# JohannesBuchner/massivedatans

Measured on AMD Instinct MI355X. Metric: likelihood evals/sec across N datasets per constrained draw, higher is better.
Workload: dtype f64

## Files before the change

### massivedatans_amd/csrc/mdns_geom.h

```cpp
#pragma once
#include "mdns_internal.h"

#ifdef __HIPCC__
#pragma clang fp contract(off)

namespace mdns {

static constexpr int kMaxRegDim = 8;
#define MDNS_DIM_SWITCH(ndim, LAUNCH) \
	switch ((ndim) <= kMaxRegDim ? (ndim) : 0) { \
	case 1: LAUNCH(1); break; case 2: LAUNCH(2); break; case 3: LAUNCH(3); break; \
	case 4: LAUNCH(4); break; case 5: LAUNCH(5); break; case 6: LAUNCH(6); break; \
	case 7: LAUNCH(7); break; case 8: LAUNCH(8); break; default: LAUNCH(0); break; }
#define MDNS_DIM5_SWITCH(ndim, LAUNCH) \
	switch (ndim) { case 1: LAUNCH(1); break; case 2: LAUNCH(2); break; case 3: LAUNCH(3); break; \
	                case 4: LAUNCH(4); break; default: LAUNCH(5); break; }

__device__ __forceinline__ double sq_distance(const double *a, const double *b, int ndim)
{
	double acc = 0.0;
	for (int k = 0; k < ndim; k++) {
		const double diff = a[k] - b[k];
		acc = acc + diff * diff;
	}
	return acc;
}

template <int D>
__device__ __forceinline__ double sq_distance_fixed(const double *a, const double (&c)[D])
{
	double acc = 0.0;
#pragma unroll
	for (int k = 0; k < D; k++) {
		const double diff = a[k] - c[k];
		acc = acc + diff * diff;
	}
	return acc;
}

__device__ __forceinline__ double wave_max(double v)
{
#pragma unroll
	for (int off = 32; off > 0; off >>= 1) v = fmax(v, __shfl_xor(v, off, 64));
	return v;
}
__device__ __forceinline__ double wave_min(double v)
{
#pragma unroll
	for (int off = 32; off > 0; off >>= 1) v = fmin(v, __shfl_xor(v, off, 64));
	return v;
}

__device__ __forceinline__ double min_or_skip(double a, double b)
{
	double r;
	asm("v_min_f64 %0, %1, %2" : "=v"(r) : "v"(a), "v"(b));
	return r;
}

__device__ __forceinline__ void atomic_max_nonneg(double *addr, double v)
{
	atomicMax(reinterpret_cast<unsigned long long *>(addr), (unsigned long long) __double_as_longlong(v));
}

template <int RT>
__device__ __forceinline__ void offer_rounds(double (&nearest)[RT], double d, unsigned m)
{
	const double PINF = __longlong_as_double(0x7ff0000000000000LL), NINF = __longlong_as_double((long long) 0xfff0000000000000ULL);
#pragma unroll
	for (int b = 0; b < RT; b++) {
		const double S = (m >> b & 1u) ? NINF : PINF;
		double t;
		asm("v_max_f64 %0, %1, %2" : "=v"(t) : "v"(d), "s"(S));
		nearest[b] = min_or_skip(nearest[b], t);
	}
}

template <int RT, bool AGENT_LOADS>
__device__ __forceinline__ void merge_chunks(const double *__restrict__ part, int K, int ny, int first_point,
                                             const unsigned *__restrict__ mask, int nb, double *__restrict__ round_sq,
                                             double (&wmax)[4][RT])
{
	const int lane = threadIdx.x & 63, wv = threadIdx.x >> 6;
	const int i = first_point + (threadIdx.x >> 2), yq = threadIdx.x & 3;
	double v[RT];
#pragma unroll
	for (int b = 0; b < RT; b++) v[b] = 0.0;
	const bool counts = i < K && i >= 1;
	if (counts) {
#pragma unroll
		for (int b = 0; b < RT; b++) v[b] = 1e300;
		for (int y = yq; y < ny; y += 4) {
			const double *row = part + ((size_t) y * K + i) * RT;
#pragma unroll
			for (int b = 0; b < RT; b++)
				v[b] = fmin(v[b], AGENT_LOADS ? __hip_atomic_load(row + b, __ATOMIC_RELAXED, __HIP_MEMORY_SCOPE_AGENT) : row[b]);
		}
	}
#pragma unroll
	for (int b = 0; b < RT; b++) {
		v[b] = fmin(v[b], __shfl_xor(v[b], 1, 64));
		v[b] = fmin(v[b], __shfl_xor(v[b], 2, 64));
	}
	if (counts) {
		const unsigned m = mask[i];
#pragma unroll
		for (int b = 0; b < RT; b++) if (b >= nb || (m >> b & 1u)) v[b] = 0.0;
	}
#pragma unroll
	for (int b = 0; b < RT; b++) {
		const double w = wave_max(v[b]);
		if (lane == 0) wmax[wv][b] = w;
	}
	__syncthreads();
	if (threadIdx.x < RT && threadIdx.x < nb) {
		const double w = fmax(fmax(wmax[0][threadIdx.x], wmax[1][threadIdx.x]), fmax(wmax[2][threadIdx.x], wmax[3][threadIdx.x]));
		if (w > 0.0) atomic_max_nonneg(round_sq + threadIdx.x, w);
	}
}

__device__ __forceinline__ void radius_and_threshold(double max_sq, double &radius, double &thresh)
{
	const double r = sqrt(max_sq);
	double T;
	if (!(r > 0.0)) T = 0.0;
	else if (r == __longlong_as_double(0x7ff0000000000000LL)) T = r;
	else {
		const double t0 = r * r;
		unsigned long long u = (unsigned long long) __double_as_longlong(t0);
		bool settled = false;
		if (t0 > 1e-300 && t0 < 1e300) {
			int guard = 0;
			while (sqrt(__longlong_as_double((long long) u)) < r && guard < 8) { u++; guard++; }
			while (guard < 16 && sqrt(__longlong_as_double((long long) (u - 1))) >= r) { u--; guard++; }
			settled = guard < 16 && sqrt(__longlong_as_double((long long) u)) >= r &&
			          sqrt(__longlong_as_double((long long) (u - 1))) < r;
		}
		if (!settled) {
			unsigned long long lo = 0, hi = 0x7ff0000000000000ULL;
			while (hi - lo > 1) {
				const unsigned long long mid = lo + (hi - lo) / 2;
				if (sqrt(__longlong_as_double((long long) mid)) >= r) hi = mid; else lo = mid;
			}
			u = hi;
		}
		T = __longlong_as_double((long long) u);
	}
	radius = r;
	thresh = T;
}

__device__ __forceinline__ void finish_radius(const BootstrapFinish &fin, double *rounds, int nrounds)
{
	if (!fin.counter) return;
	handover_release();
	__syncthreads();
	if (threadIdx.x >= 64) return;
	const int lane = threadIdx.x;
	unsigned ticket = 0;
	if (lane == 0) ticket = atomicAdd(fin.counter, 1u);
	if (__shfl(ticket, 0, 64) != gridDim.x - 1) return;
	handover_acquire();
	double best = 0.0;
	for (int b = lane; b < nrounds; b += 64)
		best = fmax(best, __hip_atomic_load(rounds + b, __ATOMIC_RELAXED, __HIP_MEMORY_SCOPE_AGENT));
	best = wave_max(best);
	for (int b = lane; b < nrounds; b += 64) rounds[b] = 0.0;
	if (lane != 0) return;
	double radius, thresh;
	radius_and_threshold(best, radius, thresh);
	fin.d_res->radius = radius;
	fin.d_res->thresh = thresh;
	*fin.counter = 0;
	mail_store(&fin.h_res->radius, radius);
	mail_store(&fin.h_res->thresh, thresh);
	mail_raise(&fin.h_res->seq, fin.seq);
}

template <int PTS>
__device__ __forceinline__ int slice_total(int hits, int *part)
{
	const int lane = threadIdx.x & 63, wv = threadIdx.x >> 6, pt = lane % PTS;
#pragma unroll
	for (int off = PTS; off < 64; off <<= 1) hits += __shfl_xor(hits, off, 64);
	if (lane < PTS) part[wv * PTS + pt] = hits;
	__syncthreads();
	return (part[pt] + part[PTS + pt]) + (part[2 * PTS + pt] + part[3 * PTS + pt]);
}

__device__ __forceinline__ void count_mail_raise(const CountMail &mail, unsigned nworkgroups)
{
	if (!mail.seq_at) return;
	if (threadIdx.x < 64) handover_release();
	__syncthreads();
	if (threadIdx.x != 0) return;
	const int done = atomicAdd(mail.ticket, 1);
	if (done != (int) nworkgroups - 1) return;
	__hip_atomic_store(mail.ticket, 0, __ATOMIC_RELAXED, __HIP_MEMORY_SCOPE_AGENT);
	mail_raise(mail.seq_at, mail.seq);
}

}
#endif
```

### massivedatans_amd/csrc/mdns_neighbors.hip

```cpp
#include "mdns_geom.h"
#include <cstdlib>
#include <cstring>

#pragma clang fp contract(off)

namespace mdns {

static constexpr int kBlock = 256;
static constexpr int kMaxTile = 512;
static constexpr int kRounds = 16;
static constexpr size_t kLdsBudget = 60 * 1024;

template <int SL> struct Geo {
	static constexpr int PTS = 64 / SL;
	static constexpr int NSLICE = 4 * SL;
};

template <typename T>
__device__ __forceinline__ void stage_to_lds(T *__restrict__ dst, const T *__restrict__ src, int count)
{
	constexpr int U = 8;
	for (int base = 0; base < count; base += U * kBlock) {
		T r[U];
#pragma unroll
		for (int u = 0; u < U; u++) {
			const int e = base + u * kBlock + (int) threadIdx.x;
			r[u] = src[e < count ? e : count - 1];
		}
#pragma unroll
		for (int u = 0; u < U; u++) {
			const int e = base + u * kBlock + (int) threadIdx.x;
			if (e < count) dst[e] = r[u];
		}
	}
}


template <int D, int SL>
__global__ __launch_bounds__(kBlock) void k_count_within(
    const double *__restrict__ members, int K, int ndim, double thresh_value,
    const RegionResult *__restrict__ res, const double *__restrict__ cands, int M,
    int *__restrict__ counts, int kchunk, int tile_n, int accumulate, CountMail mail)
{
	constexpr int PTS = Geo<SL>::PTS, NSLICE = Geo<SL>::NSLICE;
	const double thresh_sq = res ? res->thresh : thresh_value;
	extern __shared__ double smem[];
	double *tile = smem;
	int *part = reinterpret_cast<int *>(smem + (size_t) tile_n * ndim);
	const int lane = threadIdx.x & 63;
	const int wv = threadIdx.x >> 6;
	const int pt = lane % PTS;
	const int slice = wv * SL + lane / PTS;
	const int j = blockIdx.x * PTS + pt;
	const int jj = j < M ? j : M - 1;
	const int kbeg = blockIdx.y * kchunk;
	const int kend = min(K, kbeg + kchunk);

	double c[D > 0 ? D : 1];
	if (D > 0) {
#pragma unroll
		for (int k = 0; k < D; k++) c[k] = cands[(size_t) jj * D + k];
	}
	int hits = 0;
	for (int t0 = kbeg; t0 < kend; t0 += tile_n) {
		const int n = min(tile_n, kend - t0);
		__syncthreads();
		stage_to_lds(tile, members + (size_t) t0 * ndim, n * ndim);
		__syncthreads();
		if (D > 0) {
#pragma unroll 4
			for (int i = slice; i < n; i += NSLICE)
				hits += sq_distance_fixed<(D > 0 ? D : 1)>(tile + i * D, c) < thresh_sq ? 1 : 0;
		} else {
			const double *cj = cands + (size_t) jj * ndim;
			for (int i = slice; i < n; i += NSLICE)
				hits += sq_distance(tile + i * ndim, cj, ndim) < thresh_sq ? 1 : 0;
		}
	}
	const int total = slice_total<PTS>(hits, part);
	if (wv == 0 && lane < PTS && j < M) {
		if (accumulate) { if (total) atomicAdd(counts + j, total); }
		else if (mail.seq_at) __hip_atomic_store(counts + j, total, __ATOMIC_RELAXED, __HIP_MEMORY_SCOPE_SYSTEM);
		else counts[j] = total;
	}
	count_mail_raise(mail, gridDim.x * gridDim.y);
}

__global__ void k_pack_chosen(const double *__restrict__ chosen, int K, int nboot, int b0, int nb,
                              unsigned *__restrict__ mask, double *__restrict__ round_sq)
{
	const int i = blockIdx.x * blockDim.x + threadIdx.x;
	if (i < nb) round_sq[b0 + i] = 0.0;
	if (i >= K) return;
	const double *row = chosen + (size_t) i * nboot + b0;
	unsigned m = 0;
#pragma unroll
	for (int b = 0; b < kRounds; b++)
		if (b < nb) m |= (row[b] != 0.0 ? 1u : 0u) << b;
	mask[i] = m;
}

template <int D, bool NN, int SL, int RT>
__global__ __launch_bounds__(kBlock) void k_nearest_chosen(
    const double *__restrict__ members, int K, int ndim, const unsigned *__restrict__ mask,
    int nb, double *__restrict__ round_sq, int tile_n, BootstrapFinish fin, double *round_all, int nround_all,
    const double *__restrict__ chosen, int nboot, int b0)
{
	constexpr int PTS = Geo<SL>::PTS, NSLICE = Geo<SL>::NSLICE;
	constexpr int NR = NN ? 1 : RT;
	extern __shared__ double smem[];
	double *tile = smem;
	double *part = smem + (size_t) tile_n * ndim;
	unsigned *tmask = reinterpret_cast<unsigned *>(part + 4 * NR * PTS);

	const int lane = threadIdx.x & 63;
	const int wv = threadIdx.x >> 6;
	const int pt = lane % PTS;
	const int slice = wv * SL + lane / PTS;
	const int i = blockIdx.x * PTS + pt;
	const int ii = i < K ? i : K - 1;
	double c[D > 0 ? D : 1];
	if (D > 0) {
#pragma unroll
		for (int k = 0; k < D; k++) c[k] = members[(size_t) ii * D + k];
	}
	unsigned mymask = (NN || chosen) ? 0u : mask[ii];
	if (!NN && chosen) {
		const double *row = chosen + (size_t) ii * nboot + b0;
		double flag[NR];
#pragma unroll
		for (int b = 0; b < NR; b++) flag[b] = row[b < nb ? b : 0];
#pragma unroll
		for (int b = 0; b < NR; b++) mymask |= (b < nb && flag[b] != 0.0 ? 1u : 0u) << b;
	}

	double nearest[NR];
#pragma unroll
	for (int b = 0; b < NR; b++) nearest[b] = 1e300;

	for (int t0 = 0; t0 < K; t0 += tile_n) {
		const int n = min(tile_n, K - t0);
		__syncthreads();
		stage_to_lds(tile, members + (size_t) t0 * ndim, n * ndim);
		if (!NN && !chosen) stage_to_lds(tmask, mask + t0, n);
		if (!NN && chosen) {
			constexpr int TRIPS = kMaxTile / kBlock;
			double flag[TRIPS][NR];
#pragma unroll
			for (int t = 0; t < TRIPS; t++) {
				const int e = min((int) threadIdx.x + t * kBlock, n - 1);
				const double *row = chosen + (size_t) (t0 + e) * nboot + b0;
#pragma unroll
				for (int b = 0; b < NR; b++) flag[t][b] = row[b < nb ? b : 0];
			}
#pragma unroll
			for (int t = 0; t < TRIPS; t++) {
				const int e = (int) threadIdx.x + t * kBlock;
				unsigned m = 0;
#pragma unroll
				for (int b = 0; b < NR; b++) m |= (b < nb && flag[t][b] != 0.0 ? 1u : 0u) << b;
				if (e < n) tmask[e] = m;
			}
		}
		__syncthreads();
		auto offer = [&](int jn) {
			double d;
			if (D > 0) d = sq_distance_fixed<(D > 0 ? D : 1)>(tile + jn * D, c);
			else d = sq_distance(members + (size_t) ii * ndim, tile + jn * ndim, ndim);
			if (NN) {
				if (t0 + jn != ii) nearest[0] = fmin(nearest[0], d);
			} else {
				const int notchosen = (int) ~tmask[jn];
				const unsigned lo = (unsigned) __double2loint(d);
				const unsigned hi = (unsigned) __double2hiint(d);
#pragma unroll
				for (int b = 0; b < NR; b++) {
					const unsigned kill = (unsigned) __builtin_amdgcn_sbfe(notchosen, b, 1);
					const double cand = __hiloint2double((int) (hi | (kill & 0x7ff80000u)), (int) lo);
					nearest[b] = min_or_skip(nearest[b], cand);
				}
			}
		};
		int jn = slice;
		for (; jn + NSLICE < n; jn += 2 * NSLICE) {
			offer(jn);
			offer(jn + NSLICE);
		}
		if (jn < n) offer(jn);
	}
#pragma unroll
	for (int b = 0; b < NR; b++) {
		double v = nearest[b];
#pragma unroll
		for (int off = PTS; off < 64; off <<= 1) v = fmin(v, __shfl_xor(v, off, 64));
		if (lane < PTS) part[(wv * NR + b) * PTS + pt] = v;
	}
	__syncthreads();
	for (int b = wv; b < (NN ? 1 : nb); b += 4) {
		double v = 0.0;
		if (lane < PTS) {
			v = fmin(fmin(part[(0 * NR + b) * PTS + pt], part[(1 * NR + b) * PTS + pt]),
			         fmin(part[(2 * NR + b) * PTS + pt], part[(3 * NR + b) * PTS + pt]));
			const bool contributes = i < K && (NN ? true : (i >= 1 && !((mymask >> b) & 1u)));
			if (!contributes) v = 0.0;
		}
		v = wave_max(v);
		if (lane == 0 && v > 0.0) atomic_max_nonneg(round_sq + b, v);
	}
	finish_radius(fin, round_all, nround_all);
}

template <int D, int RT>
__global__ __launch_bounds__(kBlock) void k_nearest_uniform(
    const double *__restrict__ members, int K, const unsigned *__restrict__ mask, int kchunk, int tile_n,
    double *__restrict__ part, unsigned *__restrict__ block_tickets, int nb, double *__restrict__ round_sq,
    BootstrapFinish fin, int nround_all)
{
	extern __shared__ double smem[];
	double *tile = smem;
	double *meet = smem + (size_t) tile_n * D;
	unsigned *tmask = reinterpret_cast<unsigned *>(meet + 4 * RT * 64);
	const int lane = threadIdx.x & 63;
	const int wv = __builtin_amdgcn_readfirstlane(threadIdx.x >> 6);
	const int i = blockIdx.x * 64 + lane;
	const int ii = i < K ? i : K - 1;
	double c[D];
#pragma unroll
	for (int k = 0; k < D; k++) c[k] = members[(size_t) ii * D + k];
	double nearest[RT];
#pragma unroll
	for (int b = 0; b < RT; b++) nearest[b] = 1e300;
	const int kbeg = blockIdx.y * kchunk, kend = min(K, kbeg + kchunk);
	for (int t0 = kbeg; t0 < kend; t0 += tile_n) {
		const int n = min(tile_n, kend - t0);
		__syncthreads();
		stage_to_lds(tile, members + (size_t) t0 * D, n * D);
		stage_to_lds(tmask, mask + t0, n);
		__syncthreads();
		auto offer = [&](int jn) {
			const double d = sq_distance_fixed<D>(tile + jn * D, c);
			offer_rounds<RT>(nearest, d, (unsigned) __builtin_amdgcn_readfirstlane((int) tmask[jn]));
		};
		int jn = wv;
		for (; jn + 4 < n; jn += 8) { offer(jn); offer(jn + 4); }
		if (jn < n) offer(jn);
	}
#pragma unroll
	for (int b = 0; b < RT; b++) meet[(wv * RT + b) * 64 + lane] = nearest[b];
	__syncthreads();
	for (int e = threadIdx.x; e < RT * 64; e += kBlock) {
		const int b = e / 64, l = e % 64;
		const double v = fmin(fmin(meet[(0 * RT + b) * 64 + l], meet[(1 * RT + b) * 64 + l]),
		                      fmin(meet[(2 * RT + b) * 64 + l], meet[(3 * RT + b) * 64 + l]));
		const int p = blockIdx.x * 64 + l;
		if (p < K) { if (block_tickets) __hip_atomic_store(&part[((size_t) blockIdx.y * K + p) * RT + b], v, __ATOMIC_RELAXED, __HIP_MEMORY_SCOPE_AGENT); else part[((size_t) blockIdx.y * K + p) * RT + b] = v; }
	}
	if (!block_tickets) return;
	__shared__ int s_last;
	__shared__ double wmax[4][RT];
	handover_release();
	__syncthreads();
	if (threadIdx.x == 0) {
		const unsigned t = atomicAdd(block_tickets + blockIdx.x, 1u);
		s_last = t == gridDim.y - 1 ? 1 : 0;
		if (s_last) block_tickets[blockIdx.x] = 0;
	}
	__syncthreads();
	if (!s_last) return;
	handover_acquire();
	merge_chunks<RT, true>(part, K, (int) gridDim.y, blockIdx.x * 64, mask, nb, round_sq, wmax);
	finish_radius(fin, round_sq, nround_all);
}

template <int RT>
__global__ __launch_bounds__(kBlock) void k_nearest_finish(
    const double *__restrict__ part, int K, int ny, const unsigned *__restrict__ mask, int nb,
    double *__restrict__ round_sq, BootstrapFinish fin, int nround_all)
{
	__shared__ double wmax[4][RT];
	merge_chunks<RT, false>(part, K, ny, blockIdx.x * (kBlock / 4), mask, nb, round_sq, wmax);
	finish_radius(fin, round_sq, nround_all);
}

static int pick_tile(int ndim, size_t per_member_extra, size_t fixed_bytes)
{
	const size_t per = (size_t) ndim * sizeof(double) + per_member_extra;
	if (fixed_bytes + 16 * per > kLdsBudget) return 0;
	size_t n = (kLdsBudget - fixed_bytes) / per;
	if (n > (size_t) kMaxTile) n = kMaxTile;
	return (int) (n & ~(size_t) 15);
}

bool launch_count_within(const double *d_members, int K, int ndim, double thresh_sq,
                         const RegionResult *d_res, const double *d_cands, int M, int *d_counts, const CountMail *mail)
{
	Context *c = ctx();
	const CountMail none = {nullptr, nullptr, 0};
	const CountMail post = mail ? *mail : none;
	const size_t fixed = 4 * 64 * sizeof(int);
	const int tile_n = pick_tile(ndim, 0, fixed);
	if (tile_n <= 0) { set_error("ndim=%d too large for the member tile", ndim); return false; }
	const bool small = (M + 63) / 64 < 2 * c->num_cus;
	const bool fine = mail != nullptr && small;
	const int pts = fine ? 4 : (small ? 16 : 64);
	const int gx = (M + pts - 1) / pts;
	int want = (2 * c->num_cus + gx - 1) / gx;
	int max_split = (K + tile_n - 1) / tile_n;
	int gy = want < max_split ? want : max_split;
	if (mail) gy = 1;
	if (gy < 1) gy = 1;
	if (gy > 65535) gy = 65535;
	int kchunk = (K + gy - 1) / gy;
	kchunk = ((kchunk + tile_n - 1) / tile_n) * tile_n;
	gy = (K + kchunk - 1) / kchunk;
	const int accumulate = gy > 1 ? 1 : 0;
	if (accumulate && !MDNS_HIP(hipMemsetAsync(d_counts, 0, (size_t) M * sizeof(int), c->stream))) return false;
	const size_t lds = (size_t) tile_n * ndim * sizeof(double) + fixed;
	dim3 grid(gx, gy);
	ProfileScope prof(2);
#define COUNT_LAUNCH(D) do { if (fine) hipLaunchKernelGGL((k_count_within<D, 16>), grid, dim3(kBlock), lds, c->stream, \
		d_members, K, ndim, thresh_sq, d_res, d_cands, M, d_counts, kchunk, tile_n, accumulate, post); \
	else if (small) hipLaunchKernelGGL((k_count_within<D, 4>), grid, dim3(kBlock), lds, c->stream, \
		d_members, K, ndim, thresh_sq, d_res, d_cands, M, d_counts, kchunk, tile_n, accumulate, post); \
	else hipLaunchKernelGGL((k_count_within<D, 1>), grid, dim3(kBlock), lds, c->stream, \
		d_members, K, ndim, thresh_sq, d_res, d_cands, M, d_counts, kchunk, tile_n, accumulate, post); } while (0)
	MDNS_DIM_SWITCH(ndim, COUNT_LAUNCH)
#undef COUNT_LAUNCH
	return launched("k_count_within");
}

template <bool NN>
static bool launch_nearest(const double *d_members, int K, int ndim, const double *d_chosen,
                           int nboot, double *d_round_sq, const BootstrapFinish *finish,
                           const unsigned *d_packed = nullptr)
{
	Context *c = ctx();
	const bool small = (K + 63) / 64 < 2 * c->num_cus;
	const size_t fixed = (size_t) 4 * (NN ? 1 : (nboot > 10 ? kRounds : 10)) * (small ? 16 : 64) * sizeof(double);
	const int tile_n = pick_tile(ndim, sizeof(unsigned), fixed);
	if (tile_n <= 0) { set_error("ndim=%d too large for the member tile", ndim); return false; }
	const size_t lds = (size_t) tile_n * ndim * sizeof(double) + fixed + (size_t) tile_n * sizeof(unsigned);
	unsigned *d_mask = const_cast<unsigned *>(d_packed);
	if (!NN && !d_packed) {
		d_mask = (unsigned *) mask_scratch((size_t) K * sizeof(unsigned));
		if (!d_mask) return false;
	}
	const bool fused = !NN && finish && K <= 2048 && !d_packed;
	const int pts = small ? 16 : 64;
	dim3 grid((K + pts - 1) / pts);
	for (int b0 = 0; b0 < nboot; b0 += kRounds) {
		const int nb = nboot - b0 < kRounds ? nboot - b0 : kRounds;
		if (!NN && !fused && !d_packed) {
			const int nthreads = K > nb ? K : nb;
			hipLaunchKernelGGL(k_pack_chosen, dim3((nthreads + kBlock - 1) / kBlock), dim3(kBlock), 0, c->stream,
			                   d_chosen, K, nboot, b0, nb, d_mask, d_round_sq);
			if (!launched("k_pack_chosen")) return false;
		}
		BootstrapFinish fin = {nullptr, nullptr, nullptr, 0};
		if (finish && b0 + kRounds >= nboot) fin = *finish;
		ProfileScope prof(3);
#define NEAR_LAUNCH_R(D, SL, RT) hipLaunchKernelGGL((k_nearest_chosen<D, NN, SL, RT>), grid, dim3(kBlock), lds, c->stream, \
		d_members, K, ndim, d_mask, nb, d_round_sq + b0, tile_n, fin, d_round_sq, nboot, fused ? d_chosen : nullptr, nboot, b0)
#define NEAR_LAUNCH(D) do { \
	if (small) { if (NN || nb <= 10) NEAR_LAUNCH_R(D, 4, 10); else NEAR_LAUNCH_R(D, 4, kRounds); } \
	else       { if (NN || nb <= 10) NEAR_LAUNCH_R(D, 1, 10); else NEAR_LAUNCH_R(D, 1, kRounds); } } while (0)
		MDNS_DIM_SWITCH(ndim, NEAR_LAUNCH)
#undef NEAR_LAUNCH
#undef NEAR_LAUNCH_R
		if (!launched("k_nearest_chosen")) return false;
	}
	return true;
}

bool launch_bootstrap(const double *d_members, int K, int ndim, const double *d_chosen,
                      int nbootstraps, double *d_round_sq, const BootstrapFinish *finish)
{
	return launch_nearest<false>(d_members, K, ndim, d_chosen, nbootstraps, d_round_sq, finish);
}

static int uniform_chunks(int K)
{
	int most = K / 128;
	if (most < 1) most = 1;
	int best = most < 16 ? most : 16;
	static const char *forced = getenv("MDNS_K6_GY");
	if (forced && atoi(forced) > 0) best = atoi(forced) < most ? atoi(forced) : most;
	return best;
}

bool launch_bootstrap_packed(const double *d_members, int K, int ndim, const unsigned *d_packed,
                             int nbootstraps, double *d_round_sq, const BootstrapFinish *finish)
{
	if (nbootstraps > kRounds || !finish) { set_error("packed bootstrap: at most %d rounds, finishing only", kRounds); return false; }
	if (bootstrap_sorted_applies(K, ndim, nbootstraps)) return launch_bootstrap_sorted(d_members, K, ndim, d_packed, nbootstraps, d_round_sq, finish);
	Context *c = ctx();
	static const char *forced = getenv("MDNS_K6_PATH");
	const bool classic = forced && !strcmp(forced, "classic");
	if (ndim >= 1 && ndim <= 5 && K >= 640 && !classic) {
		const int rt = nbootstraps <= 10 ? 10 : kRounds;
		const int gy = uniform_chunks(K);
		int kchunk = (K + gy - 1) / gy;
		kchunk = (kchunk + 3) & ~3;
		const int ny = (K + kchunk - 1) / kchunk;
		const size_t fixed = (size_t) 4 * rt * 64 * sizeof(double);
		int tile_n = pick_tile(ndim, sizeof(unsigned), fixed);
		if (tile_n <= 0) { set_error("ndim=%d too large for the member tile", ndim); return false; }
		if (tile_n > kchunk) tile_n = (kchunk + 15) & ~15;
		const size_t lds = (size_t) tile_n * ndim * sizeof(double) + fixed + (size_t) tile_n * sizeof(unsigned);
		double *d_part = (double *) device_scratch((size_t) ny * K * rt * sizeof(double));
		if (!d_part) return false;
		dim3 grid((K + 63) / 64, ny);
		ProfileScope prof(3);
		note_kernel(3, "k_nearest_uniform<%d, %d>", ndim, rt);
		static const char *merge = getenv("MDNS_K6_MERGE");
		const bool fold = merge && !strcmp(merge, "fold");
		if (fold && !c->fold_tickets.fit_zeroed(grid.x)) return false;
		unsigned *tickets = fold ? c->fold_tickets.get() : nullptr;
#define UNI_LAUNCH(D) do { if (rt == 10) hipLaunchKernelGGL((k_nearest_uniform<D, 10>), grid, dim3(kBlock), lds, c->stream, d_members, K, d_packed, kchunk, tile_n, d_part, tickets, nbootstraps, d_round_sq, *finish, nbootstraps); \
		else hipLaunchKernelGGL((k_nearest_uniform<D, kRounds>), grid, dim3(kBlock), lds, c->stream, d_members, K, d_packed, kchunk, tile_n, d_part, tickets, nbootstraps, d_round_sq, *finish, nbootstraps); } while (0)
		MDNS_DIM5_SWITCH(ndim, UNI_LAUNCH)
#undef UNI_LAUNCH
		if (!launched("k_nearest_uniform")) return false;
		if (fold) return true;
		const dim3 fgrid((K + kBlock / 4 - 1) / (kBlock / 4));
		if (rt == 10) hipLaunchKernelGGL((k_nearest_finish<10>), fgrid, dim3(kBlock), 0, c->stream, (const double *) d_part, K, ny, d_packed, nbootstraps, d_round_sq, *finish, nbootstraps);
		else hipLaunchKernelGGL((k_nearest_finish<kRounds>), fgrid, dim3(kBlock), 0, c->stream, (const double *) d_part, K, ny, d_packed, nbootstraps, d_round_sq, *finish, nbootstraps);
		return launched("k_nearest_finish");
	}
	return launch_nearest<false>(d_members, K, ndim, nullptr, nbootstraps, d_round_sq, finish, d_packed);
}

bool launch_nn_maxsq(const double *d_members, int K, int ndim, double *d_out)
{
	return launch_nearest<true>(d_members, K, ndim, nullptr, 1, d_out, nullptr);
}

}
```

Measured before the change: 29.74 billion.

## Use finer slicing for mid-size bootstrap, fold round maxima, parallelize threshold search

For bootstrap calls with member counts in a mid range, the nearest-chosen kernel now launches with eight slices per point, which spreads each point's scan over more lanes and gives a larger grid. When the fused finish path is active, per-round maxima are folded into a single block-level atomic instead of one atomic per round per wave. The radius-threshold search now tests 64 candidate bit patterns at once across the wave using a ballot, and falls back to the serial walk only if that fails. Risks: the fold writes only round_sq[0] instead of each round slot, which changes the stored per-round values. The final wave max still covers all rounds, and the tile LDS is reused for the fold after a sync.

```diff
diff --git a/massivedatans_amd/csrc/mdns_geom.h b/massivedatans_amd/csrc/mdns_geom.h
--- a/massivedatans_amd/csrc/mdns_geom.h
+++ b/massivedatans_amd/csrc/mdns_geom.h
@@ -130,6 +130,14 @@
 		unsigned long long u = (unsigned long long) __double_as_longlong(t0);
 		bool settled = false;
 		if (t0 > 1e-300 && t0 < 1e300) {
+			const unsigned long long first = u - 32;
+			const unsigned long long pass = __ballot(sqrt(__longlong_as_double((long long) (first + (threadIdx.x & 63)))) >= r);
+			if (pass != 0 && !(pass & 1ull)) {
+				u = first + (unsigned) __builtin_ctzll(pass);
+				settled = true;
+			}
+		}
+		if (!settled && t0 > 1e-300 && t0 < 1e300) {
 			int guard = 0;
 			while (sqrt(__longlong_as_double((long long) u)) < r && guard < 8) { u++; guard++; }
 			while (guard < 16 && sqrt(__longlong_as_double((long long) (u - 1))) >= r) { u--; guard++; }
@@ -166,9 +174,9 @@
 		best = fmax(best, __hip_atomic_load(rounds + b, __ATOMIC_RELAXED, __HIP_MEMORY_SCOPE_AGENT));
 	best = wave_max(best);
 	for (int b = lane; b < nrounds; b += 64) rounds[b] = 0.0;
-	if (lane != 0) return;
 	double radius, thresh;
 	radius_and_threshold(best, radius, thresh);
+	if (lane != 0) return;
 	fin.d_res->radius = radius;
 	fin.d_res->thresh = thresh;
 	*fin.counter = 0;
diff --git a/massivedatans_amd/csrc/mdns_neighbors.hip b/massivedatans_amd/csrc/mdns_neighbors.hip
--- a/massivedatans_amd/csrc/mdns_neighbors.hip
+++ b/massivedatans_amd/csrc/mdns_neighbors.hip
@@ -15,6 +15,9 @@
 	static constexpr int PTS = 64 / SL;
 	static constexpr int NSLICE = 4 * SL;
 };
+static constexpr int kFineSL = 8;
+static constexpr int kFineFrom = 256;
+static constexpr int kFinePool = 2048;
 
 template <typename T>
 __device__ __forceinline__ void stage_to_lds(T *__restrict__ dst, const T *__restrict__ src, int count)
@@ -188,6 +191,8 @@
 		}
 		if (jn < n) offer(jn);
 	}
+	const bool fold = !NN && fin.counter != nullptr;
+	double wave_best = 0.0;
 #pragma unroll
 	for (int b = 0; b < NR; b++) {
 		double v = nearest[b];
@@ -205,7 +210,16 @@
 			if (!contributes) v = 0.0;
 		}
 		v = wave_max(v);
-		if (lane == 0 && v > 0.0) atomic_max_nonneg(round_sq + b, v);
+		if (fold) wave_best = fmax(wave_best, v);
+		else if (lane == 0 && v > 0.0) atomic_max_nonneg(round_sq + b, v);
+	}
+	if (fold) {
+		if (lane == 0) tile[wv] = wave_best;
+		__syncthreads();
+		if (threadIdx.x == 0) {
+			const double w = fmax(fmax(tile[0], tile[1]), fmax(tile[2], tile[3]));
+			if (w > 0.0) atomic_max_nonneg(round_sq, w);
+		}
 	}
 	finish_radius(fin, round_all, nround_all);
 }
@@ -336,7 +350,9 @@
 {
 	Context *c = ctx();
 	const bool small = (K + 63) / 64 < 2 * c->num_cus;
-	const size_t fixed = (size_t) 4 * (NN ? 1 : (nboot > 10 ? kRounds : 10)) * (small ? 16 : 64) * sizeof(double);
+	const bool fine = !NN && K >= kFineFrom && K <= kFinePool;
+	const int pts = fine ? 64 / kFineSL : (small ? 16 : 64);
+	const size_t fixed = (size_t) 4 * (NN ? 1 : (nboot > 10 ? kRounds : 10)) * pts * sizeof(double);
 	const int tile_n = pick_tile(ndim, sizeof(unsigned), fixed);
 	if (tile_n <= 0) { set_error("ndim=%d too large for the member tile", ndim); return false; }
 	const size_t lds = (size_t) tile_n * ndim * sizeof(double) + fixed + (size_t) tile_n * sizeof(unsigned);
@@ -346,7 +362,6 @@
 		if (!d_mask) return false;
 	}
 	const bool fused = !NN && finish && K <= 2048 && !d_packed;
-	const int pts = small ? 16 : 64;
 	dim3 grid((K + pts - 1) / pts);
 	for (int b0 = 0; b0 < nboot; b0 += kRounds) {
 		const int nb = nboot - b0 < kRounds ? nboot - b0 : kRounds;
@@ -362,7 +377,8 @@
 #define NEAR_LAUNCH_R(D, SL, RT) hipLaunchKernelGGL((k_nearest_chosen<D, NN, SL, RT>), grid, dim3(kBlock), lds, c->stream, \
 		d_members, K, ndim, d_mask, nb, d_round_sq + b0, tile_n, fin, d_round_sq, nboot, fused ? d_chosen : nullptr, nboot, b0)
 #define NEAR_LAUNCH(D) do { \
-	if (small) { if (NN || nb <= 10) NEAR_LAUNCH_R(D, 4, 10); else NEAR_LAUNCH_R(D, 4, kRounds); } \
+	if (fine)  { if (nb <= 10) NEAR_LAUNCH_R(D, (NN ? 4 : kFineSL), 10); else NEAR_LAUNCH_R(D, (NN ? 4 : kFineSL), kRounds); } \
+	else if (small) { if (NN || nb <= 10) NEAR_LAUNCH_R(D, 4, 10); else NEAR_LAUNCH_R(D, 4, kRounds); } \
 	else       { if (NN || nb <= 10) NEAR_LAUNCH_R(D, 1, 10); else NEAR_LAUNCH_R(D, 1, kRounds); } } while (0)
 		MDNS_DIM_SWITCH(ndim, NEAR_LAUNCH)
 #undef NEAR_LAUNCH
```

Result: faster. 30.78 billion (median of 6 runs) (+3.5%).
